# MVPandey/DTS

Measured on AMD Instinct MI355X. Metric: scored_trajectories_per_sec, higher is better.
Workload: dtype bf16

## Files before the change

dts_amd/ops/hip/attention.hip:

```cpp

#include "common.h"
#include "kv_cache.h"
#include <torch/extension.h>
#include <c10/hip/HIPStream.h>
#include <unordered_map>
#include <array>
#include <cstdlib>

using bf16x8 = __attribute__((ext_vector_type(8))) short;
using f32x4 = __attribute__((ext_vector_type(4))) float;
using f32x2 = __attribute__((ext_vector_type(2))) float;
using bf16x2 = __attribute__((ext_vector_type(2))) __bf16;
using u32x2 = __attribute__((ext_vector_type(2))) unsigned int;
using u32x4 = __attribute__((ext_vector_type(4))) unsigned int;


DEV bf16x8 kv_deq8(u32x2 w, float s) {
  union { bf16x2 p[4]; bf16x8 v; } c;
  c.p[0] = __builtin_amdgcn_cvt_scalef32_pk_bf16_fp8(w[0], s, false);
  c.p[1] = __builtin_amdgcn_cvt_scalef32_pk_bf16_fp8(w[0], s, true);
  c.p[2] = __builtin_amdgcn_cvt_scalef32_pk_bf16_fp8(w[1], s, false);
  c.p[3] = __builtin_amdgcn_cvt_scalef32_pk_bf16_fp8(w[1], s, true);
  return c.v;
}


template <int G, int D, typename KV = short>
__global__ void __launch_bounds__(256)
attn_decode_kernel(float* __restrict__ ws_m,
                   float* __restrict__ ws_l,
                   float* __restrict__ ws_o,
                   const short* __restrict__ q,
                   const KV* __restrict__ kcache,
                   const KV* __restrict__ vcache,
                   const int* __restrict__ block_tables,
                   const int* __restrict__ kv_lens,
                   int max_blocks, int Hkv, float scale, long q_tstride,
                   const float* __restrict__ kv_scale) {
  constexpr int BS = 16;
  constexpr int NWAVE = 4;
  constexpr int LPK = 4;
  constexpr int DPL = D / LPK;
  constexpr int DPV = D / WAVE;
  const int seq = blockIdx.x;
  const int kvh = blockIdx.y;
  const int split = blockIdx.z;
  const int S = gridDim.z;
  const int Hq = Hkv * G;
  const int wave = threadIdx.x / WAVE;
  const int lane = threadIdx.x & (WAVE - 1);
  const int kv_len = kv_lens[seq];
  const int n_pages = (kv_len + BS - 1) / BS;
  const int pages_per_split = (n_pages + S - 1) / S;
  const int page_lo = split * pages_per_split;
  const int page_hi = min(n_pages, page_lo + pages_per_split);
  const long ws_base = (((long)seq * Hkv + kvh) * S + split) * G;
  if (page_lo >= page_hi) {
    for (int g = threadIdx.x; g < G; g += blockDim.x) {
      ws_m[ws_base + g] = -1e30f;
      ws_l[ws_base + g] = 0.f;
    }
    return;
  }

  __shared__ float s_scores[NWAVE][G][BS];
  __shared__ float s_m[NWAVE][G], s_l[NWAVE][G];
  __shared__ float s_o[NWAVE][G][D];

  const int c = lane & (LPK - 1);
  const int key_of_lane = lane / LPK;
  int qp_[G][DPL / 2];
#pragma unroll
  for (int g = 0; g < G; ++g) {
    const short* qp = q + (long)seq * q_tstride + (long)(kvh * G + g) * D + c * DPL;
#pragma unroll
    for (int i = 0; i < DPL / 2; ++i) qp_[g][i] = ((const int*)qp)[i];
  }

  float m[G], lsum[G], o[G][DPV];
#pragma unroll
  for (int g = 0; g < G; ++g) {
    m[g] = -1e30f;
    lsum[g] = 0.f;
#pragma unroll
    for (int d = 0; d < DPV; ++d) o[g][d] = 0.f;
  }

  const int* bt = block_tables + (long)seq * max_blocks;

  float sscale = scale;
  if constexpr (sizeof(KV) == 1) {
    if (kv_scale) sscale *= kv_scale[kvh];
  }

  for (int page = page_lo + wave; page < page_hi; page += NWAVE) {
    const long blk = bt[page];
    const KV* kbase =
        kcache + ((blk * Hkv + kvh) * BS) * (long)D;
    const KV* vbase =
        vcache + ((blk * Hkv + kvh) * BS) * (long)D;
    const int valid = min(BS, kv_len - page * BS);

    float partial[G];
#pragma unroll
    for (int g = 0; g < G; ++g) partial[g] = 0.f;
    if constexpr (sizeof(KV) == 1) {
      if (key_of_lane < valid) {
        const KV* kp = kbase + key_of_lane * D + c * DPL;
        unsigned int kw[DPL / 4];
#pragma unroll
        for (int x = 0; x < DPL / 16; ++x) {
          const u32x4 t = ((const u32x4*)kp)[x];
#pragma unroll
          for (int y = 0; y < 4; ++y) kw[4 * x + y] = t[y];
        }
#pragma unroll
        for (int w = 0; w < DPL / 4; ++w) {
          const f32x2 kf[2] = {
              __builtin_amdgcn_cvt_pk_f32_fp8((int)kw[w], false),
              __builtin_amdgcn_cvt_pk_f32_fp8((int)kw[w], true)};
#pragma unroll
          for (int h = 0; h < 2; ++h) {
            const int i = 2 * w + h;
            float k0 = kf[h][0];
            float k1 = kf[h][1];
#pragma unroll
            for (int g = 0; g < G; ++g) {
              float q0 = bf2f((short)(qp_[g][i] & 0xffff));
              float q1 = bf2f((short)((qp_[g][i] >> 16) & 0xffff));
              partial[g] += q0 * k0 + q1 * k1;
            }
          }
        }
      }
    } else if (key_of_lane < valid) {
      const KV* kp = kbase + key_of_lane * D + c * DPL;
#pragma unroll
      for (int i = 0; i < DPL / 2; ++i) {
        int kw = ((const int*)kp)[i];
        float k0 = bf2f((short)(kw & 0xffff));
        float k1 = bf2f((short)((kw >> 16) & 0xffff));
#pragma unroll
        for (int g = 0; g < G; ++g) {
          float q0 = bf2f((short)(qp_[g][i] & 0xffff));
          float q1 = bf2f((short)((qp_[g][i] >> 16) & 0xffff));
          partial[g] += q0 * k0 + q1 * k1;
        }
      }
    }
#pragma unroll
    for (int g = 0; g < G; ++g) {
      partial[g] += __shfl_xor(partial[g], 1, 64);
      partial[g] += __shfl_xor(partial[g], 2, 64);
      if (c == 0)
        s_scores[wave][g][key_of_lane] =
            (key_of_lane < valid) ? partial[g] * sscale : -1e30f;
    }
    asm volatile("s_waitcnt lgkmcnt(0)" ::: "memory");
    __builtin_amdgcn_wave_barrier();

    int vw[BS];
#pragma unroll
    for (int j = 0; j < BS; ++j) {
      if (j < valid) {
        if constexpr (sizeof(KV) == 1) {
          if constexpr (DPV == 2)
            vw[j] = (int)*(const unsigned short*)(vbase + j * D + 2 * lane);
          else
            vw[j] = (int)*(const unsigned char*)(vbase + j * D + lane);
        } else if constexpr (DPV == 2) {
          vw[j] = *(const int*)(vbase + j * D + 2 * lane);
        } else {
          vw[j] = (int)*(const unsigned short*)(vbase + j * D + lane);
        }
      } else {
        vw[j] = 0;
      }
    }

#pragma unroll
    for (int g = 0; g < G; ++g) {
      float tmax = -1e30f;
#pragma unroll
      for (int j = 0; j < BS; ++j) tmax = fmaxf(tmax, s_scores[wave][g][j]);
      float m_new = fmaxf(m[g], tmax);
      if (m_new > -1e30f) {
        float alpha = __expf(m[g] - m_new);
#pragma unroll
        for (int d = 0; d < DPV; ++d) o[g][d] *= alpha;
        lsum[g] *= alpha;
        m[g] = m_new;
        float p[BS];
        float psum = 0.f;
#pragma unroll
        for (int j = 0; j < BS; ++j) {
          p[j] = (j < valid) ? __expf(s_scores[wave][g][j] - m_new) : 0.f;
          psum += p[j];
        }
        lsum[g] += psum;
        if constexpr (sizeof(KV) == 1) {
#pragma unroll
          for (int j = 0; j < BS; ++j) {
            const f32x2 vf = __builtin_amdgcn_cvt_pk_f32_fp8(vw[j], false);
            o[g][0] += p[j] * vf[0];
            if constexpr (DPV == 2) o[g][1] += p[j] * vf[1];
          }
        } else {
#pragma unroll
          for (int j = 0; j < BS; ++j) {
            o[g][0] += p[j] * bf2f((short)(vw[j] & 0xffff));
            if constexpr (DPV == 2)
              o[g][1] += p[j] * bf2f((short)((vw[j] >> 16) & 0xffff));
          }
        }
      }
    }
    __builtin_amdgcn_wave_barrier();
  }

#pragma unroll
  for (int g = 0; g < G; ++g) {
    if (lane == 0) {
      s_m[wave][g] = m[g];
      s_l[wave][g] = lsum[g];
    }
#pragma unroll
    for (int d = 0; d < DPV; ++d) s_o[wave][g][lane * DPV + d] = o[g][d];
  }
  __syncthreads();

  float vscale = 1.f;
  if constexpr (sizeof(KV) == 1) {
    if (kv_scale) vscale = kv_scale[Hkv + kvh];
  }
  const int tid = threadIdx.x;
  for (int gd = tid; gd < G * (D / 2); gd += blockDim.x) {
    const int g = gd / (D / 2);
    const int d0 = (gd % (D / 2)) * 2;
    float m_star = -1e30f;
#pragma unroll
    for (int w = 0; w < NWAVE; ++w) m_star = fmaxf(m_star, s_m[w][g]);
    float l_star = 0.f, acc0 = 0.f, acc1 = 0.f;
#pragma unroll
    for (int w = 0; w < NWAVE; ++w) {
      float f = (s_m[w][g] > -1e30f) ? __expf(s_m[w][g] - m_star) : 0.f;
      l_star += s_l[w][g] * f;
      acc0 += s_o[w][g][d0] * f;
      acc1 += s_o[w][g][d0 + 1] * f;
    }
    if (d0 == 0) {
      ws_m[ws_base + g] = m_star;
      ws_l[ws_base + g] = l_star;
    }
    float* wo = ws_o + (ws_base + g) * D;
    if constexpr (sizeof(KV) == 1) {
      wo[d0] = acc0 * vscale;
      wo[d0 + 1] = acc1 * vscale;
    } else {
      wo[d0] = acc0;
      wo[d0 + 1] = acc1;
    }
  }
}

template <int D>
__global__ void __launch_bounds__(256)
attn_decode_combine(short* __restrict__ out,
                    const float* __restrict__ ws_m,
                    const float* __restrict__ ws_l,
                    const float* __restrict__ ws_o,
                    int S, int G, int Hkv) {
  const int seq = blockIdx.x;
  const int hq = blockIdx.y;
  const int kvh = hq / G;
  const int g = hq % G;
  const int Hq = Hkv * G;
  const long base0 = (((long)seq * Hkv + kvh) * S) * G + g;

  __shared__ float sh_f[64];
  __shared__ float sh_linv[1];
  if (threadIdx.x == 0) {
    float m_star = -1e30f;
    for (int s2 = 0; s2 < S; ++s2)
      m_star = fmaxf(m_star, ws_m[base0 + (long)s2 * G]);
    float l_star = 0.f;
    for (int s2 = 0; s2 < S; ++s2) {
      float mm = ws_m[base0 + (long)s2 * G];
      float f = (mm > -1e30f) ? __expf(mm - m_star) : 0.f;
      sh_f[s2] = f;
      l_star += ws_l[base0 + (long)s2 * G] * f;
    }
    sh_linv[0] = (l_star > 0.f) ? 1.f / l_star : 0.f;
  }
  __syncthreads();
  const float linv = sh_linv[0];
  for (int d = threadIdx.x; d < D; d += blockDim.x) {
    float acc = 0.f;
    for (int s2 = 0; s2 < S; ++s2) {
      float f = sh_f[s2];
      if (f > 0.f) acc += ws_o[(base0 + (long)s2 * G) * D + d] * f;
    }
    out[(((long)seq * Hq) + hq) * D + d] = f2bf(acc * linv);
  }
}


template <int G, int D, int KSTEP>
__global__ void __launch_bounds__(256)
attn_prefill_kernel_v2(short* __restrict__ out,
                       const short* __restrict__ q,
                       const int* __restrict__ cu_q,
                       const long* __restrict__ q_pos,
                       const short* __restrict__ kcache,
                       const short* __restrict__ vcache,
                       const int* __restrict__ block_tables,
                       const int* __restrict__ kv_lens, int max_blocks,
                       int Hkv, float scale, long q_tstride) {
  constexpr int BS = 16;
  constexpr int KCHUNKS = D / 32;
  constexpr int CTILES = D / 16;
  constexpr int LDK = D + 8;
  constexpr int LDV = KSTEP + 4;
  constexpr int ROWS = 64;
  const int POS_PER_WG = ROWS / G;

  const int seq = blockIdx.y;
  const int kvh = blockIdx.z;
  const int Hq = Hkv * G;
  const int q_start = cu_q[seq];
  const int q_len = cu_q[seq + 1] - q_start;
  const int tile = blockIdx.x;
  if (tile * POS_PER_WG >= q_len) return;

  const int wave = threadIdx.x / WAVE;
  const int lane = threadIdx.x & (WAVE - 1);
  const int kv_len = kv_lens[seq];
  const int* bt = block_tables + (long)seq * max_blocks;

  __shared__ short k_lds[KSTEP][LDK];
  __shared__ short v_lds_t[D][LDV];
  __shared__ float s_scores[4][16][KSTEP];
  __shared__ float s_alpha[4][16];
  __shared__ float s_rowl[4][16];
  __shared__ short p_lds[4][16][KSTEP];

  short a_frag[KCHUNKS][8];
  {
    const int r = lane & 15;
    const int row_global = wave * 16 + r;
    const int pos_local = tile * POS_PER_WG + row_global / G;
    const int head = row_global % G;
    const bool valid_row = pos_local < q_len;
    const int tok = q_start + (valid_row ? pos_local : 0);
    const short* qp = q + (long)tok * q_tstride + (long)(kvh * G + head) * D;
#pragma unroll
    for (int kc = 0; kc < KCHUNKS; ++kc) {
      const int kbase = kc * 32 + (lane >> 4) * 8;
      bf16x8 v8 = *(const bf16x8*)(qp + kbase);
#pragma unroll
      for (int i = 0; i < 8; ++i)
        a_frag[kc][i] = valid_row ? v8[i] : (short)0;
    }
  }
  constexpr int SMW = KSTEP / 4;
  const int sm_row = lane / 4;
  const int sm_sub = lane & 3;
  const long sm_pos = tile * POS_PER_WG + (wave * 16 + sm_row) / G;
  const bool sm_valid = sm_pos < q_len;
  const long sm_abs_pos = sm_valid ? q_pos[q_start + sm_pos] : -1;

  f32x4 o_acc[CTILES];
#pragma unroll
  for (int ct = 0; ct < CTILES; ++ct) o_acc[ct] = {0.f, 0.f, 0.f, 0.f};
  float run_m = -1e30f, run_l = 0.f;

  const int last_local_pos = min(q_len, tile * POS_PER_WG + POS_PER_WG) - 1;
  const long last_abs_pos = q_pos[q_start + last_local_pos];
  const int kv_hi = min((long)kv_len, last_abs_pos + 1);

  constexpr int CHUNKS_PT = KSTEP * D / (256 * 8);
  bf16x8 k_stage[CHUNKS_PT], v_stage[CHUNKS_PT];
  int st_key[CHUNKS_PT], st_d0[CHUNKS_PT];

  auto issue_tile = [&](int kv_base) {
#pragma unroll
    for (int c = 0; c < CHUNKS_PT; ++c) {
      const int base = (threadIdx.x + c * 256) * 8;
      const int key = base / D;
      const int d0 = base % D;
      st_key[c] = key;
      st_d0[c] = d0;
      const int kglob = kv_base + key;
      if (kglob < kv_len) {
        const long blk = bt[kglob / BS];
        const long off = ((blk * Hkv + kvh) * BS + kglob % BS) * (long)D + d0;
        k_stage[c] = *(const bf16x8*)(kcache + off);
        v_stage[c] = *(const bf16x8*)(vcache + off);
      } else {
        const bf16x8 z = {0, 0, 0, 0, 0, 0, 0, 0};
        k_stage[c] = z;
        v_stage[c] = z;
      }
    }
  };
  auto write_tile = [&]() {
#pragma unroll
    for (int c = 0; c < CHUNKS_PT; ++c) {
      *(bf16x8*)(&k_lds[st_key[c]][st_d0[c]]) = k_stage[c];
#pragma unroll
      for (int i = 0; i < 8; ++i)
        v_lds_t[st_d0[c] + i][st_key[c]] = v_stage[c][i];
    }
  };

  issue_tile(0);
  write_tile();
  __syncthreads();

  for (int kv_base = 0; kv_base < kv_hi; kv_base += KSTEP) {
    const int kv_next = kv_base + KSTEP;
    if (kv_next < kv_hi) issue_tile(kv_next);

#pragma unroll
    for (int st = 0; st < KSTEP / 16; ++st) {
      f32x4 acc = {0.f, 0.f, 0.f, 0.f};
#pragma unroll
      for (int kc = 0; kc < KCHUNKS; ++kc) {
        const int key = st * 16 + (lane & 15);
        const int d0 = kc * 32 + (lane >> 4) * 8;
        bf16x8 b8 = *(bf16x8*)(&k_lds[key][d0]);
        acc = __builtin_amdgcn_mfma_f32_16x16x32_bf16(
            *(bf16x8*)a_frag[kc], b8, acc, 0, 0, 0);
      }
#pragma unroll
      for (int i = 0; i < 4; ++i) {
        const int row = (lane >> 4) * 4 + i;
        s_scores[wave][row][st * 16 + (lane & 15)] = acc[i] * scale;
      }
    }
    __builtin_amdgcn_s_waitcnt(0);
    __builtin_amdgcn_wave_barrier();

    {
      float tmax = -1e30f;
      float sc[SMW];
#pragma unroll
      for (int jj = 0; jj < SMW; ++jj) {
        const int j = sm_sub * SMW + jj;
        const long key_abs = kv_base + j;
        float s = s_scores[wave][sm_row][j];
        const bool ok =
            sm_valid && key_abs <= sm_abs_pos && key_abs < (long)kv_len;
        sc[jj] = ok ? s : -1e30f;
        tmax = fmaxf(tmax, sc[jj]);
      }
      tmax = fmaxf(tmax, __shfl_xor(tmax, 1, 64));
      tmax = fmaxf(tmax, __shfl_xor(tmax, 2, 64));
      float m_new = fmaxf(run_m, tmax);
      float alpha, rowsum = 0.f;
      if (m_new > -1e30f) {
        alpha = (run_m > -1e30f) ? __expf(run_m - m_new) : 0.f;
#pragma unroll
        for (int jj = 0; jj < SMW; ++jj) {
          float p = (sc[jj] > -1e30f) ? __expf(sc[jj] - m_new) : 0.f;
          p_lds[wave][sm_row][sm_sub * SMW + jj] = f2bf(p);
          rowsum += p;
        }
      } else {
        alpha = 1.f;
#pragma unroll
        for (int jj = 0; jj < SMW; ++jj)
          p_lds[wave][sm_row][sm_sub * SMW + jj] = 0;
      }
      rowsum += __shfl_xor(rowsum, 1, 64);
      rowsum += __shfl_xor(rowsum, 2, 64);
      run_l = run_l * alpha + rowsum;
      run_m = m_new;
      if (sm_sub == 0) {
        s_alpha[wave][sm_row] = alpha;
        s_rowl[wave][sm_row] = run_l;
      }
    }
    __builtin_amdgcn_s_waitcnt(0);
    __builtin_amdgcn_wave_barrier();

    {
      float al[4];
#pragma unroll
      for (int i = 0; i < 4; ++i) al[i] = s_alpha[wave][(lane >> 4) * 4 + i];
      constexpr int HCH = KSTEP / 32;
      bf16x8 pa[HCH];
      {
        const int row = lane & 15;
#pragma unroll
        for (int h = 0; h < HCH; ++h) {
          const int k0 = h * 32 + (lane >> 4) * 8;
#pragma unroll
          for (int i = 0; i < 8; ++i) pa[h][i] = p_lds[wave][row][k0 + i];
        }
      }
#pragma unroll
      for (int ct = 0; ct < CTILES; ++ct) {
#pragma unroll
        for (int i = 0; i < 4; ++i) o_acc[ct][i] *= al[i];
        const int dim = ct * 16 + (lane & 15);
#pragma unroll
        for (int h = 0; h < HCH; ++h) {
          const int kk0 = h * 32 + (lane >> 4) * 8;
          bf16x8 vb;
          ((unsigned long long*)&vb)[0] =
              *(const unsigned long long*)(&v_lds_t[dim][kk0]);
          ((unsigned long long*)&vb)[1] =
              *(const unsigned long long*)(&v_lds_t[dim][kk0 + 4]);
          o_acc[ct] = __builtin_amdgcn_mfma_f32_16x16x32_bf16(
              pa[h], vb, o_acc[ct], 0, 0, 0);
        }
      }
    }
    __syncthreads();
    if (kv_next < kv_hi) {
      write_tile();
      __syncthreads();
    }
  }

  {
    float invl[4];
#pragma unroll
    for (int i = 0; i < 4; ++i) {
      float l = s_rowl[wave][(lane >> 4) * 4 + i];
      invl[i] = (l > 0.f) ? 1.f / l : 0.f;
    }
#pragma unroll
    for (int ct = 0; ct < CTILES; ++ct) {
#pragma unroll
      for (int i = 0; i < 4; ++i) {
        const int row = (lane >> 4) * 4 + i;
        const int row_global = wave * 16 + row;
        const int pos_local = tile * POS_PER_WG + row_global / G;
        if (pos_local >= q_len) continue;
        const int head = row_global % G;
        const int tok = q_start + pos_local;
        const int dim = ct * 16 + (lane & 15);
        out[((long)tok * Hq + kvh * G + head) * D + dim] =
            f2bf(o_acc[ct][i] * invl[i]);
      }
    }
  }
}


template <int G, int D, int KSTEP, typename KV = short>
__global__ void __launch_bounds__(256)
attn_prefill_kernel_v5(short* __restrict__ out,
                       const short* __restrict__ q,
                       const int* __restrict__ cu_q,
                       const long* __restrict__ q_pos,
                       const KV* __restrict__ kcache,
                       const KV* __restrict__ vcache,
                       const int* __restrict__ block_tables,
                       const int* __restrict__ kv_lens, int max_blocks,
                       int Hkv, float scale, long q_tstride,
                       const float* __restrict__ kv_scale) {
  constexpr int BS = 16;
  constexpr int KCHUNKS = D / 32;
  constexpr int CTILES = D / 16;
  constexpr int LDS_PAD = 8;
  constexpr int LDK = D + LDS_PAD;
  constexpr int ROWS = 64;
  const int POS_PER_WG = ROWS / G;

  const int seq = blockIdx.y;
  const int kvh = blockIdx.z;
  const int Hq = Hkv * G;
  const int q_start = cu_q[seq];
  const int q_len = cu_q[seq + 1] - q_start;
  const int tile = blockIdx.x;
  if (tile * POS_PER_WG >= q_len) return;

  const int wave = threadIdx.x / WAVE;
  const int lane = threadIdx.x & (WAVE - 1);
  const int kv_len = kv_lens[seq];
  const int* bt = block_tables + (long)seq * max_blocks;

  __shared__ short k_lds[KSTEP][LDK];
  __shared__ short v_lds[KSTEP][LDK];

  float k_scale = 1.f, v_scale = 1.f;
  if constexpr (sizeof(KV) == 1) {
    if (kv_scale) {
      k_scale = kv_scale[kvh];
      v_scale = kv_scale[Hkv + kvh];
    }
  }

  short q_frag[KCHUNKS][8];
  {
    const int r = lane & 15;
    const int row_global = wave * 16 + r;
    const int pos_local = tile * POS_PER_WG + row_global / G;
    const int head = row_global % G;
    const bool valid_row = pos_local < q_len;
    const int tok = q_start + (valid_row ? pos_local : 0);
    const short* qp = q + (long)tok * q_tstride + (long)(kvh * G + head) * D;
#pragma unroll
    for (int kc = 0; kc < KCHUNKS; ++kc) {
      const int kbase = kc * 32 + (lane >> 4) * 8;
      bf16x8 v8 = *(const bf16x8*)(qp + kbase);
#pragma unroll
      for (int i = 0; i < 8; ++i)
        q_frag[kc][i] = valid_row ? v8[i] : (short)0;
    }
  }
  const int my_q = lane & 15;
  const int my_row_global = wave * 16 + my_q;
  const long my_pos_local = tile * POS_PER_WG + my_row_global / G;
  const bool my_valid = my_pos_local < q_len;
  const long my_abs_pos = my_valid ? q_pos[q_start + my_pos_local] : -1;

  f32x4 o_acc[CTILES];
#pragma unroll
  for (int ct = 0; ct < CTILES; ++ct) o_acc[ct] = {0.f, 0.f, 0.f, 0.f};
  float run_m = -1e30f, run_l = 0.f;

  const int last_local_pos = min(q_len, tile * POS_PER_WG + POS_PER_WG) - 1;
  const long last_abs_pos = q_pos[q_start + last_local_pos];
  const int kv_hi = min((long)kv_len, last_abs_pos + 1);

  for (int kv_base = 0; kv_base < kv_hi; kv_base += KSTEP) {
    {
      const int elems = KSTEP * D;
      for (int base = threadIdx.x * 8; base < elems; base += 256 * 8) {
        const int key = base / D;
        const int d0 = base % D;
        const int kglob = kv_base + key;
        if (kglob < kv_len) {
          const long blk = bt[kglob / BS];
          const long off =
              ((blk * Hkv + kvh) * BS + kglob % BS) * (long)D + d0;
          if constexpr (sizeof(KV) == 1) {
            *(bf16x8*)(&k_lds[key][d0]) =
                kv_deq8(*(const u32x2*)(kcache + off), k_scale);
            *(bf16x8*)(&v_lds[key][d0]) =
                kv_deq8(*(const u32x2*)(vcache + off), v_scale);
          } else {
            *(bf16x8*)(&k_lds[key][d0]) = *(const bf16x8*)(kcache + off);
            *(bf16x8*)(&v_lds[key][d0]) = *(const bf16x8*)(vcache + off);
          }
        } else {
          const bf16x8 z = {0, 0, 0, 0, 0, 0, 0, 0};
          *(bf16x8*)(&k_lds[key][d0]) = z;
          *(bf16x8*)(&v_lds[key][d0]) = z;
        }
      }
    }
    __syncthreads();

    constexpr int STILES = KSTEP / 16;
    f32x4 sc[STILES];
#pragma unroll
    for (int st = 0; st < STILES; ++st) {
      f32x4 acc = {0.f, 0.f, 0.f, 0.f};
#pragma unroll
      for (int kc = 0; kc < KCHUNKS; ++kc) {
        const int key = st * 16 + (lane & 15);
        const int d0 = kc * 32 + (lane >> 4) * 8;
        bf16x8 k8 = *(bf16x8*)(&k_lds[key][d0]);
        acc = __builtin_amdgcn_mfma_f32_16x16x32_bf16(
            k8, *(bf16x8*)q_frag[kc], acc, 0, 0, 0);
      }
      sc[st] = acc;
    }

    float p[STILES][4];
    float tmax = -1e30f;
#pragma unroll
    for (int st = 0; st < STILES; ++st)
#pragma unroll
      for (int i = 0; i < 4; ++i) {
        const long key_abs = kv_base + st * 16 + (lane >> 4) * 4 + i;
        const bool ok =
            my_valid && key_abs <= my_abs_pos && key_abs < (long)kv_len;
        p[st][i] = ok ? sc[st][i] * scale : -1e30f;
        tmax = fmaxf(tmax, p[st][i]);
      }
    tmax = fmaxf(tmax, __shfl_xor(tmax, 16, 64));
    tmax = fmaxf(tmax, __shfl_xor(tmax, 32, 64));
    const float m_new = fmaxf(run_m, tmax);
    float alpha;
    float rowsum = 0.f;
    if (m_new > -1e30f) {
      alpha = (run_m > -1e30f) ? __expf(run_m - m_new) : 0.f;
#pragma unroll
      for (int st = 0; st < STILES; ++st)
#pragma unroll
        for (int i = 0; i < 4; ++i) {
          p[st][i] = (p[st][i] > -1e30f) ? __expf(p[st][i] - m_new) : 0.f;
          rowsum += p[st][i];
        }
    } else {
      alpha = 1.f;
#pragma unroll
      for (int st = 0; st < STILES; ++st)
#pragma unroll
        for (int i = 0; i < 4; ++i) p[st][i] = 0.f;
    }
    rowsum += __shfl_xor(rowsum, 16, 64);
    rowsum += __shfl_xor(rowsum, 32, 64);
    run_l = run_l * alpha + rowsum;
    run_m = m_new;

    unsigned int ppack[STILES][2];
#pragma unroll
    for (int st = 0; st < STILES; ++st) {
#pragma unroll
      for (int hpair = 0; hpair < 2; ++hpair) {
        const unsigned int lo =
            (unsigned short)f2bf(p[st][hpair * 2]);
        const unsigned int hi =
            (unsigned short)f2bf(p[st][hpair * 2 + 1]);
        ppack[st][hpair] = lo | (hi << 16);
      }
    }
    constexpr int HCH = KSTEP / 32;
    bf16x8 pa[HCH];
#pragma unroll
    for (int h = 0; h < HCH; ++h) {
      const int kb = 8 * (lane >> 4);
      const int st_a = h * 2 + kb / 16;
      const int ga = (kb % 16) / 4;
      const int st_b = h * 2 + (kb + 4) / 16;
      const int gb = ((kb + 4) % 16) / 4;
      unsigned int paw[4];
#pragma unroll
      for (int pr = 0; pr < 2; ++pr) {
        unsigned int va = 0, vb2 = 0;
#pragma unroll
        for (int st = 0; st < STILES; ++st) {
          const unsigned int ta =
              (unsigned int)__shfl((int)ppack[st][pr], (ga << 4) | my_q, 64);
          const unsigned int tb =
              (unsigned int)__shfl((int)ppack[st][pr], (gb << 4) | my_q, 64);
          if (st == st_a) va = ta;
          if (st == st_b) vb2 = tb;
        }
        paw[pr] = va;
        paw[2 + pr] = vb2;
      }
#pragma unroll
      for (int j = 0; j < 4; ++j) {
        pa[h][2 * j] = (short)(paw[j] & 0xffff);
        pa[h][2 * j + 1] = (short)(paw[j] >> 16);
      }
    }
#pragma unroll
    for (int ct = 0; ct < CTILES; ++ct) {
#pragma unroll
      for (int i = 0; i < 4; ++i) {
        const float al = __shfl(alpha, (lane >> 4) * 4 + i, 64);
        o_acc[ct][i] *= al;
      }
    }
#pragma unroll
    for (int ct = 0; ct < CTILES; ++ct) {
      const int dim = ct * 16 + (lane & 15);
#pragma unroll
      for (int h = 0; h < HCH; ++h) {
        bf16x8 vb;
        const int kk0 = h * 32 + (lane >> 4) * 8;
#pragma unroll
        for (int i = 0; i < 8; ++i) vb[i] = v_lds[kk0 + i][dim];
        o_acc[ct] = __builtin_amdgcn_mfma_f32_16x16x32_bf16(
            pa[h], vb, o_acc[ct], 0, 0, 0);
      }
    }
    __syncthreads();
  }

  {
#pragma unroll
    for (int ct = 0; ct < CTILES; ++ct) {
#pragma unroll
      for (int i = 0; i < 4; ++i) {
        const int row = (lane >> 4) * 4 + i;
        const float l = __shfl(run_l, row, 64);
        const float invl = (l > 0.f) ? 1.f / l : 0.f;
        const int row_global = wave * 16 + row;
        const int pos_local = tile * POS_PER_WG + row_global / G;
        if (pos_local >= q_len) continue;
        const int head = row_global % G;
        const int tok = q_start + pos_local;
        const int dim = ct * 16 + (lane & 15);
        out[((long)tok * Hq + kvh * G + head) * D + dim] =
            f2bf(o_acc[ct][i] * invl);
      }
    }
  }
}


template <int G, int D, bool SWZ, typename KV = short>
__global__ void __launch_bounds__(256)
attn_prefill_kernel(short* __restrict__ out,
                    const short* __restrict__ q,
                    const int* __restrict__ cu_q,
                    const long* __restrict__ q_pos,
                    const KV* __restrict__ kcache,
                    const KV* __restrict__ vcache,
                    const int* __restrict__ block_tables,
                    const int* __restrict__ kv_lens, int max_blocks, int Hkv,
                    float scale, long q_tstride,
                    const float* __restrict__ kv_scale) {
  constexpr int BS = 16;
  constexpr int KSTEP = 32;
  constexpr int KCHUNKS = D / 32;
  constexpr int CTILES = D / 16;
  constexpr int LDS_PAD = 8;
  constexpr int LDK = D + LDS_PAD;
  constexpr int ROWS = 64;
  const int POS_PER_WG = ROWS / G;

  const int seq = blockIdx.y;
  const int kvh = blockIdx.z;
  const int Hq = Hkv * G;
  const int q_start = cu_q[seq];
  const int q_len = cu_q[seq + 1] - q_start;
  const int tile = blockIdx.x;
  if (tile * POS_PER_WG >= q_len) return;

  const int wave = threadIdx.x / WAVE;
  const int lane = threadIdx.x & (WAVE - 1);
  const int kv_len = kv_lens[seq];
  const int* bt = block_tables + (long)seq * max_blocks;

  __shared__ short k_lds[KSTEP][LDK];
  __shared__ short v_lds[KSTEP][LDK];
  float k_scale = 1.f, v_scale = 1.f;
  if constexpr (sizeof(KV) == 1) {
    if (kv_scale) {
      k_scale = kv_scale[kvh];
      v_scale = kv_scale[Hkv + kvh];
    }
  }
  auto swz_col = [](int key, int col) -> int {
    if constexpr (SWZ) return ((col & ~7) ^ ((key & 7) << 3)) | (col & 7);
    else return col;
  };
  __shared__ float s_scores[4][16][KSTEP];
  __shared__ float s_alpha[4][16];
  __shared__ float s_rowl[4][16];
  __shared__ short p_lds[4][16][KSTEP];

  long my_pos[4];
  short a_frag[KCHUNKS][8];
  {
    const int r = lane & 15;
    const int row_global = wave * 16 + r;
    const int pos_local = tile * POS_PER_WG + row_global / G;
    const int head = row_global % G;
    const bool valid_row = pos_local < q_len;
    const int tok = q_start + (valid_row ? pos_local : 0);
    const short* qp = q + (long)tok * q_tstride + (long)(kvh * G + head) * D;
#pragma unroll
    for (int kc = 0; kc < KCHUNKS; ++kc) {
      const int kbase = kc * 32 + (lane >> 4) * 8;
      bf16x8 v8 = *(const bf16x8*)(qp + kbase);
#pragma unroll
      for (int i = 0; i < 8; ++i)
        a_frag[kc][i] = valid_row ? v8[i] : (short)0;
    }
  }
  const int sm_row = lane / 4;
  const int sm_sub = lane & 3;
  const long sm_pos =
      tile * POS_PER_WG + (wave * 16 + sm_row) / G;
  const bool sm_valid = sm_pos < q_len;
  const long sm_abs_pos = sm_valid ? q_pos[q_start + sm_pos] : -1;

  f32x4 o_acc[CTILES];
#pragma unroll
  for (int ct = 0; ct < CTILES; ++ct) o_acc[ct] = {0.f, 0.f, 0.f, 0.f};
  float run_m = -1e30f, run_l = 0.f;

  const int last_local_pos = min(q_len, tile * POS_PER_WG + POS_PER_WG) - 1;
  const long last_abs_pos = q_pos[q_start + last_local_pos];
  const int kv_hi = min((long)kv_len, last_abs_pos + 1);

  for (int kv_base = 0; kv_base < kv_hi; kv_base += KSTEP) {
    {
      const int elems = KSTEP * D;
      for (int base = threadIdx.x * 8; base < elems; base += 256 * 8) {
        const int key = base / D;
        const int d0 = base % D;
        const int page = kv_base / BS + key / BS;
        const int koff = key % BS;
        const int kglob = kv_base + key;
        const int dst = swz_col(key, d0);
        if (kglob < kv_len) {
          const long blk = bt[page];
          const KV* kp =
              kcache + ((blk * Hkv + kvh) * BS + koff) * (long)D + d0;
          const KV* vp =
              vcache + ((blk * Hkv + kvh) * BS + koff) * (long)D + d0;
          if constexpr (sizeof(KV) == 1) {
            *(bf16x8*)(&k_lds[key][dst]) = kv_deq8(*(const u32x2*)kp, k_scale);
            *(bf16x8*)(&v_lds[key][dst]) = kv_deq8(*(const u32x2*)vp, v_scale);
          } else {
            *(bf16x8*)(&k_lds[key][dst]) = *(const bf16x8*)kp;
            *(bf16x8*)(&v_lds[key][dst]) = *(const bf16x8*)vp;
          }
        } else {
          bf16x8 z = {0, 0, 0, 0, 0, 0, 0, 0};
          *(bf16x8*)(&k_lds[key][dst]) = z;
          *(bf16x8*)(&v_lds[key][dst]) = z;
        }
      }
    }
    __syncthreads();

#pragma unroll
    for (int st = 0; st < 2; ++st) {
      f32x4 acc = {0.f, 0.f, 0.f, 0.f};
#pragma unroll
      for (int kc = 0; kc < KCHUNKS; ++kc) {
        const int key = st * 16 + (lane & 15);
        const int d0 = kc * 32 + (lane >> 4) * 8;
        bf16x8 b8 = *(const bf16x8*)(&k_lds[key][swz_col(key, d0)]);
        acc = __builtin_amdgcn_mfma_f32_16x16x32_bf16(
            *(bf16x8*)a_frag[kc], b8, acc, 0, 0, 0);
      }
#pragma unroll
      for (int i = 0; i < 4; ++i) {
        const int row = (lane >> 4) * 4 + i;
        s_scores[wave][row][st * 16 + (lane & 15)] = acc[i] * scale;
      }
    }
    __builtin_amdgcn_s_waitcnt(0);
    __builtin_amdgcn_wave_barrier();

    {
      float tmax = -1e30f;
      float sc[8];
#pragma unroll
      for (int jj = 0; jj < 8; ++jj) {
        const int j = sm_sub * 8 + jj;
        const long key_abs = kv_base + j;
        float s = s_scores[wave][sm_row][j];
        const bool ok = sm_valid && key_abs <= sm_abs_pos &&
                        key_abs < (long)kv_len;
        sc[jj] = ok ? s : -1e30f;
        tmax = fmaxf(tmax, sc[jj]);
      }
      tmax = fmaxf(tmax, __shfl_xor(tmax, 1, 64));
      tmax = fmaxf(tmax, __shfl_xor(tmax, 2, 64));
      float m_new = fmaxf(run_m, tmax);
      float alpha, rowsum = 0.f;
      if (m_new > -1e30f) {
        alpha = (run_m > -1e30f) ? __expf(run_m - m_new) : 0.f;
#pragma unroll
        for (int jj = 0; jj < 8; ++jj) {
          float p = (sc[jj] > -1e30f) ? __expf(sc[jj] - m_new) : 0.f;
          p_lds[wave][sm_row][sm_sub * 8 + jj] = f2bf(p);
          rowsum += p;
        }
      } else {
        alpha = 1.f;
#pragma unroll
        for (int jj = 0; jj < 8; ++jj)
          p_lds[wave][sm_row][sm_sub * 8 + jj] = 0;
      }
      rowsum += __shfl_xor(rowsum, 1, 64);
      rowsum += __shfl_xor(rowsum, 2, 64);
      run_l = run_l * alpha + rowsum;
      run_m = m_new;
      if (sm_sub == 0) {
        s_alpha[wave][sm_row] = alpha;
        s_rowl[wave][sm_row] = run_l;
      }
    }
    __builtin_amdgcn_s_waitcnt(0);
    __builtin_amdgcn_wave_barrier();

    {
      float al[4];
#pragma unroll
      for (int i = 0; i < 4; ++i) al[i] = s_alpha[wave][(lane >> 4) * 4 + i];
      bf16x8 pa0, pa1;
      {
        const int row = lane & 15;
        const int k0 = (lane >> 4) * 8;
#pragma unroll
        for (int i = 0; i < 8; ++i) pa0[i] = p_lds[wave][row][k0 + i];
        pa1 = pa0;
      }
#pragma unroll
      for (int ct = 0; ct < CTILES; ++ct) {
#pragma unroll
        for (int i = 0; i < 4; ++i) o_acc[ct][i] *= al[i];
        bf16x8 vb;
        const int dim = ct * 16 + (lane & 15);
        const int kk0 = (lane >> 4) * 8;
#pragma unroll
        for (int i = 0; i < 8; ++i)
          vb[i] = v_lds[kk0 + i][swz_col(kk0 + i, dim)];
        o_acc[ct] = __builtin_amdgcn_mfma_f32_16x16x32_bf16(pa0, vb,
                                                            o_acc[ct], 0, 0, 0);
      }
    }
    __syncthreads();
  }

  {
    float invl[4];
#pragma unroll
    for (int i = 0; i < 4; ++i) {
      float l = s_rowl[wave][(lane >> 4) * 4 + i];
      invl[i] = (l > 0.f) ? 1.f / l : 0.f;
    }
#pragma unroll
    for (int ct = 0; ct < CTILES; ++ct) {
#pragma unroll
      for (int i = 0; i < 4; ++i) {
        const int row = (lane >> 4) * 4 + i;
        const int row_global = wave * 16 + row;
        const int pos_local = tile * POS_PER_WG + row_global / G;
        if (pos_local >= q_len) continue;
        const int head = row_global % G;
        const int tok = q_start + pos_local;
        const int dim = ct * 16 + (lane & 15);
        out[((long)tok * Hq + kvh * G + head) * D + dim] =
            f2bf(o_acc[ct][i] * invl[i]);
      }
    }
  }
}


void attn_decode_paged(torch::Tensor out, torch::Tensor q,
                       torch::Tensor kcache, torch::Tensor vcache,
                       torch::Tensor block_tables, torch::Tensor kv_lens,
                       double scale, c10::optional<torch::Tensor> kv_scale) {
  const int B = q.size(0), Hq = q.size(1), D = q.size(2);
  const int Hkv = kcache.size(1);
  const int G = Hq / Hkv;
  const int max_blocks = block_tables.size(1);
  TORCH_CHECK(kcache.size(2) == 16, "block_size must be 16");
  const bool fp8 = kv_cache_is_fp8(kcache, vcache);
  const float* kv_scale_p = kv_scale_ptr(kv_scale, kcache, fp8);
  TORCH_CHECK(block_tables.scalar_type() == torch::kInt32);
  TORCH_CHECK(q.stride(2) == 1 && q.stride(1) == D, "q heads must be dense");
  TORCH_CHECK(out.is_contiguous(), "out must be contiguous");
  const long q_tstride = q.stride(0);
  static const int S = [] {
    const char* e = getenv("DTS_DECODE_SPLITS");
    int v = e ? atoi(e) : 8;
    return (v >= 1 && v <= 64) ? v : 8;
  }();
  static std::unordered_map<std::string, std::array<torch::Tensor, 3>> ws_cache;
  const std::string key = std::to_string(q.get_device()) + ":" +
                          std::to_string(B) + ":" + std::to_string(Hkv) + ":" +
                          std::to_string(G) + ":" + std::to_string(D);
  auto it = ws_cache.find(key);
  if (it == ws_cache.end()) {
    auto f32 =
        torch::TensorOptions().dtype(torch::kFloat32).device(q.device());
    it = ws_cache
             .emplace(key,
                      std::array<torch::Tensor, 3>{
                          torch::empty({B, Hkv, S, G}, f32),
                          torch::empty({B, Hkv, S, G}, f32),
                          torch::empty({(long)B, Hkv, S, G, D}, f32)})
             .first;
  }
  torch::Tensor ws_m = it->second[0];
  torch::Tensor ws_l = it->second[1];
  torch::Tensor ws_o = it->second[2];
  dim3 grid(B, Hkv, S);
  dim3 block(256);
  auto stream = c10::hip::getCurrentHIPStream();
#define DECODE_LAUNCH(g, d, kv)                                              \
  hipLaunchKernelGGL((attn_decode_kernel<g, d, kv>), grid, block, 0, stream, \
                     (float*)ws_m.data_ptr(), (float*)ws_l.data_ptr(),       \
                     (float*)ws_o.data_ptr(), (const short*)q.data_ptr(),    \
                     (const kv*)kcache.data_ptr(),                           \
                     (const kv*)vcache.data_ptr(),                           \
                     (const int*)block_tables.data_ptr(),                    \
                     (const int*)kv_lens.data_ptr(), max_blocks, Hkv,        \
                     (float)scale, q_tstride, kv_scale_p)
#define DECODE_CASE(g, d)                                                    \
  do {                                                                       \
    if (fp8) DECODE_LAUNCH(g, d, unsigned char);                             \
    else DECODE_LAUNCH(g, d, short);                                         \
    hipLaunchKernelGGL((attn_decode_combine<d>), dim3(B, Hq), dim3(256), 0,  \
                       stream, (short*)out.data_ptr(),                       \
                       (const float*)ws_m.data_ptr(),                        \
                       (const float*)ws_l.data_ptr(),                        \
                       (const float*)ws_o.data_ptr(), S, G, Hkv);            \
  } while (0)
  if (D == 128 && G == 4) DECODE_CASE(4, 128);
  else if (D == 128 && G == 8) DECODE_CASE(8, 128);
  else if (D == 128 && G == 1) DECODE_CASE(1, 128);
  else if (D == 64 && G == 1) DECODE_CASE(1, 64);
  else TORCH_CHECK(false, "unsupported decode attn shape D=", D, " G=", G);
#undef DECODE_CASE
#undef DECODE_LAUNCH
  HIP_CHECK_LAST();
}

void attn_prefill_paged(torch::Tensor out, torch::Tensor q, torch::Tensor cu_q,
                        torch::Tensor q_pos, torch::Tensor kcache,
                        torch::Tensor vcache, torch::Tensor block_tables,
                        torch::Tensor kv_lens, double scale, int64_t swz,
                        c10::optional<torch::Tensor> kv_scale) {
  if (swz < 0) {
    static int env_v = [] {
      const char* e = getenv("DTS_PREFILL_V");
      return e ? atoi(e) : -1;
    }();
    swz = (env_v >= 0) ? env_v : 5;
  }
  const bool fp8 = kv_cache_is_fp8(kcache, vcache);
  TORCH_CHECK(!fp8 || swz == 0 || swz == 4 || swz == 5,
              "prefill variant ", swz, " (DTS_PREFILL_V) does not support an "
              "FP8 KV cache; use 0, 4 or 5");
  const float* kv_scale_p = kv_scale_ptr(kv_scale, kcache, fp8);
  const int Hq = q.size(1), D = q.size(2);
  const int Hkv = kcache.size(1);
  const int G = Hq / Hkv;
  const int P = cu_q.size(0) - 1;
  const int max_blocks = block_tables.size(1);
  TORCH_CHECK(q.stride(2) == 1 && q.stride(1) == D, "q heads must be dense");
  TORCH_CHECK(out.is_contiguous(), "out must be contiguous");
  const long q_tstride = q.stride(0);
  TORCH_CHECK(D == 128 || D == 64, "prefill kernel supports head_dim 64/128");
  TORCH_CHECK(kcache.size(2) == 16, "block_size must be 16");
  TORCH_CHECK(cu_q.scalar_type() == torch::kInt32);
  const long Tq = q.size(0);
  const int pos_per_wg = 64 / G;
  const int max_tiles = (int)((Tq + pos_per_wg - 1) / pos_per_wg);
  dim3 grid(max_tiles, P, Hkv);
  dim3 block(256);
  auto stream = c10::hip::getCurrentHIPStream();
#define PREFILL_CASE(g, d)                                                    \
  do {                                                                        \
    if (swz == 2)                                                             \
      hipLaunchKernelGGL((attn_prefill_kernel_v2<g, d, 64>), grid, block, 0,  \
                         stream, (short*)out.data_ptr(),                      \
                         (const short*)q.data_ptr(),                          \
                         (const int*)cu_q.data_ptr(),                         \
                         (const long*)q_pos.data_ptr(),                       \
                         (const short*)kcache.data_ptr(),                     \
                         (const short*)vcache.data_ptr(),                     \
                         (const int*)block_tables.data_ptr(),                 \
                         (const int*)kv_lens.data_ptr(), max_blocks, Hkv,     \
                         (float)scale, q_tstride);                            \
    else if (swz == 3)                                                        \
      hipLaunchKernelGGL((attn_prefill_kernel_v2<g, d, 32>), grid, block, 0,  \
                         stream, (short*)out.data_ptr(),                      \
                         (const short*)q.data_ptr(),                          \
                         (const int*)cu_q.data_ptr(),                         \
                         (const long*)q_pos.data_ptr(),                       \
                         (const short*)kcache.data_ptr(),                     \
                         (const short*)vcache.data_ptr(),                     \
                         (const int*)block_tables.data_ptr(),                 \
                         (const int*)kv_lens.data_ptr(), max_blocks, Hkv,     \
                         (float)scale, q_tstride);                            \
    else if (swz == 4)                                                        \
      hipLaunchKernelGGL((attn_prefill_kernel_v5<g, d, 32>), grid, block, 0,  \
                         stream, (short*)out.data_ptr(),                      \
                         (const short*)q.data_ptr(),                         \
                         (const int*)cu_q.data_ptr(),                         \
                         (const long*)q_pos.data_ptr(),                       \
                         (const short*)kcache.data_ptr(),                     \
                         (const short*)vcache.data_ptr(),                     \
                         (const int*)block_tables.data_ptr(),                 \
                         (const int*)kv_lens.data_ptr(), max_blocks, Hkv,     \
                         (float)scale, q_tstride, nullptr);                   \
    else if (swz == 5)                                                        \
      hipLaunchKernelGGL((attn_prefill_kernel_v5<g, d, 64>), grid, block, 0,  \
                         stream, (short*)out.data_ptr(),                      \
                         (const short*)q.data_ptr(),                         \
                         (const int*)cu_q.data_ptr(),                         \
                         (const long*)q_pos.data_ptr(),                       \
                         (const short*)kcache.data_ptr(),                     \
                         (const short*)vcache.data_ptr(),                     \
                         (const int*)block_tables.data_ptr(),                 \
                         (const int*)kv_lens.data_ptr(), max_blocks, Hkv,     \
                         (float)scale, q_tstride, nullptr);                   \
    else if (swz == 1)                                                        \
      hipLaunchKernelGGL((attn_prefill_kernel<g, d, true>), grid, block, 0,   \
                         stream, (short*)out.data_ptr(),                      \
                         (const short*)q.data_ptr(),                          \
                         (const int*)cu_q.data_ptr(),                         \
                         (const long*)q_pos.data_ptr(),                       \
                         (const short*)kcache.data_ptr(),                     \
                         (const short*)vcache.data_ptr(),                     \
                         (const int*)block_tables.data_ptr(),                 \
                         (const int*)kv_lens.data_ptr(), max_blocks, Hkv,     \
                         (float)scale, q_tstride, nullptr);                   \
    else                                                                      \
      hipLaunchKernelGGL((attn_prefill_kernel<g, d, false>), grid, block, 0,  \
                         stream, (short*)out.data_ptr(),                      \
                         (const short*)q.data_ptr(),                          \
                         (const int*)cu_q.data_ptr(),                         \
                         (const long*)q_pos.data_ptr(),                       \
                         (const short*)kcache.data_ptr(),                     \
                         (const short*)vcache.data_ptr(),                     \
                         (const int*)block_tables.data_ptr(),                 \
                         (const int*)kv_lens.data_ptr(), max_blocks, Hkv,     \
                         (float)scale, q_tstride, nullptr);                   \
  } while (0)
#define PREFILL_LAUNCH_FP8(kern)                                              \
  hipLaunchKernelGGL(kern, grid, block, 0, stream, (short*)out.data_ptr(),    \
                     (const short*)q.data_ptr(), (const int*)cu_q.data_ptr(), \
                     (const long*)q_pos.data_ptr(),                           \
                     (const unsigned char*)kcache.data_ptr(),                 \
                     (const unsigned char*)vcache.data_ptr(),                 \
                     (const int*)block_tables.data_ptr(),                     \
                     (const int*)kv_lens.data_ptr(), max_blocks, Hkv,         \
                     (float)scale, q_tstride, kv_scale_p)
#define PREFILL_CASE_FP8(g, d)                                                \
  do {                                                                        \
    if (swz == 4)                                                             \
      PREFILL_LAUNCH_FP8((attn_prefill_kernel_v5<g, d, 32, unsigned char>));  \
    else if (swz == 5)                                                        \
      PREFILL_LAUNCH_FP8((attn_prefill_kernel_v5<g, d, 64, unsigned char>));  \
    else                                                                      \
      PREFILL_LAUNCH_FP8((attn_prefill_kernel<g, d, false, unsigned char>));  \
  } while (0)
  if (fp8) {
    if (D == 128 && G == 4) PREFILL_CASE_FP8(4, 128);
    else if (D == 128 && G == 8) PREFILL_CASE_FP8(8, 128);
    else if (D == 128 && G == 1) PREFILL_CASE_FP8(1, 128);
    else if (D == 128 && G == 2) PREFILL_CASE_FP8(2, 128);
    else if (D == 64 && G == 1) PREFILL_CASE_FP8(1, 64);
    else TORCH_CHECK(false, "unsupported prefill shape G=", G, " D=", D);
  } else if (D == 128 && G == 4) PREFILL_CASE(4, 128);
  else if (D == 128 && G == 8) PREFILL_CASE(8, 128);
  else if (D == 128 && G == 1) PREFILL_CASE(1, 128);
  else if (D == 128 && G == 2) PREFILL_CASE(2, 128);
  else if (D == 64 && G == 1) PREFILL_CASE(1, 64);
  else TORCH_CHECK(false, "unsupported prefill shape G=", G, " D=", D);
#undef PREFILL_CASE
#undef PREFILL_CASE_FP8
#undef PREFILL_LAUNCH_FP8
  HIP_CHECK_LAST();
}
```

Baseline: 0.3868.

## Add v6 prefill attention kernel with register prefetch and transposed LDS V reads

Adds a new paged prefill attention kernel, v6, and makes it the default variant. It double-buffers KV tile loads through registers: the next tile's global loads and block-table lookups are issued before the current tile's compute, and the data is committed to LDS afterward. V is stored in grouped LDS rows and read with ds_read_tr16_b64 transpose loads instead of element-wise gathers. This hides global memory latency and cuts LDS read instructions, at the cost of more registers per thread and a second sync per iteration.

```diff
diff --git a/dts_amd/ops/hip/attention.hip b/dts_amd/ops/hip/attention.hip
--- a/dts_amd/ops/hip/attention.hip
+++ b/dts_amd/ops/hip/attention.hip
@@ -775,6 +775,334 @@
       }
     }
     __syncthreads();
+  }
+
+  {
+#pragma unroll
+    for (int ct = 0; ct < CTILES; ++ct) {
+#pragma unroll
+      for (int i = 0; i < 4; ++i) {
+        const int row = (lane >> 4) * 4 + i;
+        const float l = __shfl(run_l, row, 64);
+        const float invl = (l > 0.f) ? 1.f / l : 0.f;
+        const int row_global = wave * 16 + row;
+        const int pos_local = tile * POS_PER_WG + row_global / G;
+        if (pos_local >= q_len) continue;
+        const int head = row_global % G;
+        const int tok = q_start + pos_local;
+        const int dim = ct * 16 + (lane & 15);
+        out[((long)tok * Hq + kvh * G + head) * D + dim] =
+            f2bf(o_acc[ct][i] * invl);
+      }
+    }
+  }
+}
+
+
+typedef short i16x4 __attribute__((ext_vector_type(4)));
+typedef __attribute__((address_space(3))) i16x4 lds_i16x4;
+
+template <int G, int D, int KSTEP, typename KV = short, bool PF = false>
+__global__ void __launch_bounds__(256)
+attn_prefill_kernel_v6(short* __restrict__ out,
+                       const short* __restrict__ q,
+                       const int* __restrict__ cu_q,
+                       const long* __restrict__ q_pos,
+                       const KV* __restrict__ kcache,
+                       const KV* __restrict__ vcache,
+                       const int* __restrict__ block_tables,
+                       const int* __restrict__ kv_lens, int max_blocks,
+                       int Hkv, float scale, long q_tstride,
+                       const float* __restrict__ kv_scale) {
+  static_assert(KSTEP == 64, "v6 is built for 64-key tiles");
+  constexpr int BS = 16;
+  constexpr int KCHUNKS = D / 32;
+  constexpr int CTILES = D / 16;
+  constexpr int LDS_PAD = 8;
+  constexpr int LDK = D + LDS_PAD;
+  constexpr int LDV = D + 16;
+  constexpr int VGRP = 8 * LDV + 64;
+  constexpr int ROWS = 64;
+  constexpr int NIT = KSTEP * D / (256 * 8);
+  constexpr int KEYS_PER_IT = 256 * 8 / D;
+  constexpr bool FP8 = sizeof(KV) == 1;
+  const int POS_PER_WG = ROWS / G;
+
+  const int seq = blockIdx.y;
+  const int kvh = blockIdx.z;
+  const int Hq = Hkv * G;
+  const int q_start = cu_q[seq];
+  const int q_len = cu_q[seq + 1] - q_start;
+  const int tile = blockIdx.x;
+  if (tile * POS_PER_WG >= q_len) return;
+
+  const int wave = threadIdx.x / WAVE;
+  const int lane = threadIdx.x & (WAVE - 1);
+  const int kv_len = kv_lens[seq];
+  const int* bt = block_tables + (long)seq * max_blocks;
+
+  __shared__ __attribute__((aligned(16))) short k_lds[KSTEP][LDK];
+  __shared__ __attribute__((aligned(16))) short v_lds[(KSTEP / 8) * VGRP];
+  auto v_off = [](int key, int col) -> int {
+    return (key >> 3) * VGRP + (key & 7) * LDV + col;
+  };
+
+  float k_scale = 1.f, v_scale = 1.f;
+  if constexpr (FP8) {
+    if (kv_scale) {
+      k_scale = kv_scale[kvh];
+      v_scale = kv_scale[Hkv + kvh];
+    }
+  }
+
+  short q_frag[KCHUNKS][8];
+  {
+    const int r = lane & 15;
+    const int row_global = wave * 16 + r;
+    const int pos_local = tile * POS_PER_WG + row_global / G;
+    const int head = row_global % G;
+    const bool valid_row = pos_local < q_len;
+    const int tok = q_start + (valid_row ? pos_local : 0);
+    const short* qp = q + (long)tok * q_tstride + (long)(kvh * G + head) * D;
+#pragma unroll
+    for (int kc = 0; kc < KCHUNKS; ++kc) {
+      const int kbase = kc * 32 + (lane >> 4) * 8;
+      bf16x8 v8 = *(const bf16x8*)(qp + kbase);
+#pragma unroll
+      for (int i = 0; i < 8; ++i)
+        q_frag[kc][i] = valid_row ? v8[i] : (short)0;
+    }
+  }
+  const int my_q = lane & 15;
+  const int my_row_global = wave * 16 + my_q;
+  const long my_pos_local = tile * POS_PER_WG + my_row_global / G;
+  const bool my_valid = my_pos_local < q_len;
+  const long my_abs_pos = my_valid ? q_pos[q_start + my_pos_local] : -1;
+
+  f32x4 o_acc[CTILES];
+#pragma unroll
+  for (int ct = 0; ct < CTILES; ++ct) o_acc[ct] = {0.f, 0.f, 0.f, 0.f};
+  float run_m = -1e30f, run_l = 0.f;
+
+  const int last_local_pos = min(q_len, tile * POS_PER_WG + POS_PER_WG) - 1;
+  const long last_abs_pos = q_pos[q_start + last_local_pos];
+  const int kv_hi = min((long)kv_len, last_abs_pos + 1);
+
+  const int ld_key = threadIdx.x * 8 / D;
+  const int ld_d0 = threadIdx.x * 8 % D;
+  const short* v_rd =
+      &v_lds[v_off(8 * (lane >> 4) + ((lane >> 2) & 3), 4 * (lane & 3))];
+
+  using stage_t = typename std::conditional<FP8, u32x2, bf16x8>::type;
+  stage_t kreg[NIT], vreg[NIT];
+  int blk_next[NIT];
+  auto fetch_bt = [&](int base) {
+#pragma unroll
+    for (int it = 0; it < NIT; ++it) {
+      const int kg = min(base + ld_key + it * KEYS_PER_IT, kv_len - 1);
+      blk_next[it] = bt[kg / BS];
+    }
+  };
+  auto issue_tile = [&](int base) {
+#pragma unroll
+    for (int it = 0; it < NIT; ++it) {
+      const int kg = min(base + ld_key + it * KEYS_PER_IT, kv_len - 1);
+      const long off =
+          (((long)blk_next[it] * Hkv + kvh) * BS + kg % BS) * (long)D + ld_d0;
+      kreg[it] = *(const stage_t*)(kcache + off);
+      vreg[it] = *(const stage_t*)(vcache + off);
+    }
+  };
+  auto commit_tile = [&](int base) {
+#pragma unroll
+    for (int it = 0; it < NIT; ++it) {
+      const int key = ld_key + it * KEYS_PER_IT;
+      const bool live = base + key < kv_len;
+      bf16x8 k8, v8;
+      if constexpr (FP8) {
+        k8 = kv_deq8(kreg[it], k_scale);
+        v8 = kv_deq8(vreg[it], v_scale);
+      } else {
+        k8 = kreg[it];
+        v8 = vreg[it];
+      }
+      const bf16x8 z = {0, 0, 0, 0, 0, 0, 0, 0};
+      *(bf16x8*)(&k_lds[key][ld_d0]) = live ? k8 : z;
+      *(bf16x8*)(&v_lds[v_off(key, ld_d0)]) = live ? v8 : z;
+    }
+  };
+
+  if constexpr (PF) {
+    if (kv_hi > 0) {
+      fetch_bt(0);
+      issue_tile(0);
+      if (KSTEP < kv_hi) fetch_bt(KSTEP);
+      commit_tile(0);
+      __syncthreads();
+    }
+  }
+
+  for (int kv_base = 0; kv_base < kv_hi; kv_base += KSTEP) {
+    if constexpr (PF) {
+      if (kv_base + KSTEP < kv_hi) {
+        issue_tile(kv_base + KSTEP);
+        if (kv_base + 2 * KSTEP < kv_hi) fetch_bt(kv_base + 2 * KSTEP);
+      }
+    } else {
+      const int elems = KSTEP * D;
+      for (int base = threadIdx.x * 8; base < elems; base += 256 * 8) {
+        const int key = base / D;
+        const int d0 = base % D;
+        const int kglob = kv_base + key;
+        if (kglob < kv_len) {
+          const long blk = bt[kglob / BS];
+          const long off =
+              ((blk * Hkv + kvh) * BS + kglob % BS) * (long)D + d0;
+          if constexpr (sizeof(KV) == 1) {
+            *(bf16x8*)(&k_lds[key][d0]) =
+                kv_deq8(*(const u32x2*)(kcache + off), k_scale);
+            *(bf16x8*)(&v_lds[v_off(key, d0)]) =
+                kv_deq8(*(const u32x2*)(vcache + off), v_scale);
+          } else {
+            *(bf16x8*)(&k_lds[key][d0]) = *(const bf16x8*)(kcache + off);
+            *(bf16x8*)(&v_lds[v_off(key, d0)]) =
+                *(const bf16x8*)(vcache + off);
+          }
+        } else {
+          const bf16x8 z = {0, 0, 0, 0, 0, 0, 0, 0};
+          *(bf16x8*)(&k_lds[key][d0]) = z;
+          *(bf16x8*)(&v_lds[v_off(key, d0)]) = z;
+        }
+      }
+      __syncthreads();
+    }
+
+    constexpr int STILES = KSTEP / 16;
+    f32x4 sc[STILES];
+#pragma unroll
+    for (int st = 0; st < STILES; ++st) {
+      f32x4 acc = {0.f, 0.f, 0.f, 0.f};
+#pragma unroll
+      for (int kc = 0; kc < KCHUNKS; ++kc) {
+        const int key = st * 16 + (lane & 15);
+        const int d0 = kc * 32 + (lane >> 4) * 8;
+        bf16x8 k8 = *(bf16x8*)(&k_lds[key][d0]);
+        acc = __builtin_amdgcn_mfma_f32_16x16x32_bf16(
+            k8, *(bf16x8*)q_frag[kc], acc, 0, 0, 0);
+      }
+      sc[st] = acc;
+    }
+
+    float p[STILES][4];
+    float tmax = -1e30f;
+#pragma unroll
+    for (int st = 0; st < STILES; ++st)
+#pragma unroll
+      for (int i = 0; i < 4; ++i) {
+        const long key_abs = kv_base + st * 16 + (lane >> 4) * 4 + i;
+        const bool ok =
+            my_valid && key_abs <= my_abs_pos && key_abs < (long)kv_len;
+        p[st][i] = ok ? sc[st][i] * scale : -1e30f;
+        tmax = fmaxf(tmax, p[st][i]);
+      }
+    tmax = fmaxf(tmax, __shfl_xor(tmax, 16, 64));
+    tmax = fmaxf(tmax, __shfl_xor(tmax, 32, 64));
+    const float m_new = fmaxf(run_m, tmax);
+    float alpha;
+    float rowsum = 0.f;
+    if (m_new > -1e30f) {
+      alpha = (run_m > -1e30f) ? __expf(run_m - m_new) : 0.f;
+#pragma unroll
+      for (int st = 0; st < STILES; ++st)
+#pragma unroll
+        for (int i = 0; i < 4; ++i) {
+          p[st][i] = (p[st][i] > -1e30f) ? __expf(p[st][i] - m_new) : 0.f;
+          rowsum += p[st][i];
+        }
+    } else {
+      alpha = 1.f;
+#pragma unroll
+      for (int st = 0; st < STILES; ++st)
+#pragma unroll
+        for (int i = 0; i < 4; ++i) p[st][i] = 0.f;
+    }
+    rowsum += __shfl_xor(rowsum, 16, 64);
+    rowsum += __shfl_xor(rowsum, 32, 64);
+    run_l = run_l * alpha + rowsum;
+    run_m = m_new;
+
+    unsigned int ppack[STILES][2];
+#pragma unroll
+    for (int st = 0; st < STILES; ++st) {
+#pragma unroll
+      for (int hpair = 0; hpair < 2; ++hpair) {
+        const unsigned int lo =
+            (unsigned short)f2bf(p[st][hpair * 2]);
+        const unsigned int hi =
+            (unsigned short)f2bf(p[st][hpair * 2 + 1]);
+        ppack[st][hpair] = lo | (hi << 16);
+      }
+    }
+    constexpr int HCH = KSTEP / 32;
+    bf16x8 pa[HCH];
+#pragma unroll
+    for (int h = 0; h < HCH; ++h) {
+      const int kb = 8 * (lane >> 4);
+      const int st_a = h * 2 + kb / 16;
+      const int ga = (kb % 16) / 4;
+      const int st_b = h * 2 + (kb + 4) / 16;
+      const int gb = ((kb + 4) % 16) / 4;
+      unsigned int paw[4];
+#pragma unroll
+      for (int pr = 0; pr < 2; ++pr) {
+        unsigned int va = 0, vb2 = 0;
+#pragma unroll
+        for (int st = 0; st < STILES; ++st) {
+          const unsigned int ta =
+              (unsigned int)__shfl((int)ppack[st][pr], (ga << 4) | my_q, 64);
+          const unsigned int tb =
+              (unsigned int)__shfl((int)ppack[st][pr], (gb << 4) | my_q, 64);
+          if (st == st_a) va = ta;
+          if (st == st_b) vb2 = tb;
+        }
+        paw[pr] = va;
+        paw[2 + pr] = vb2;
+      }
+#pragma unroll
+      for (int j = 0; j < 4; ++j) {
+        pa[h][2 * j] = (short)(paw[j] & 0xffff);
+        pa[h][2 * j + 1] = (short)(paw[j] >> 16);
+      }
+    }
+#pragma unroll
+    for (int ct = 0; ct < CTILES; ++ct) {
+#pragma unroll
+      for (int i = 0; i < 4; ++i) {
+        const float al = __shfl(alpha, (lane >> 4) * 4 + i, 64);
+        o_acc[ct][i] *= al;
+      }
+    }
+#pragma unroll
+    for (int ct = 0; ct < CTILES; ++ct) {
+#pragma unroll
+      for (int h = 0; h < HCH; ++h) {
+        const short* vp = v_rd + h * 4 * VGRP + ct * 16;
+        const i16x4 lo =
+            __builtin_amdgcn_ds_read_tr16_b64_v4i16((lds_i16x4*)vp);
+        const i16x4 hi = __builtin_amdgcn_ds_read_tr16_b64_v4i16(
+            (lds_i16x4*)(vp + 4 * LDV));
+        const bf16x8 vb = __builtin_shufflevector(lo, hi, 0, 1, 2, 3, 4, 5, 6, 7);
+        o_acc[ct] = __builtin_amdgcn_mfma_f32_16x16x32_bf16(
+            pa[h], vb, o_acc[ct], 0, 0, 0);
+      }
+    }
+    __syncthreads();
+    if constexpr (PF) {
+      if (kv_base + KSTEP < kv_hi) {
+        commit_tile(kv_base + KSTEP);
+        __syncthreads();
+      }
+    }
   }
 
   {
@@ -1117,12 +1445,13 @@
       const char* e = getenv("DTS_PREFILL_V");
       return e ? atoi(e) : -1;
     }();
-    swz = (env_v >= 0) ? env_v : 5;
+    swz = (env_v >= 0) ? env_v : 6;
   }
   const bool fp8 = kv_cache_is_fp8(kcache, vcache);
-  TORCH_CHECK(!fp8 || swz == 0 || swz == 4 || swz == 5,
+  const bool v6 = swz == 6 || swz == 7;
+  TORCH_CHECK(!fp8 || swz == 0 || swz == 4 || swz == 5 || v6,
               "prefill variant ", swz, " (DTS_PREFILL_V) does not support an "
-              "FP8 KV cache; use 0, 4 or 5");
+              "FP8 KV cache; use 0, 4, 5, 6 or 7");
   const float* kv_scale_p = kv_scale_ptr(kv_scale, kcache, fp8);
   const int Hq = q.size(1), D = q.size(2);
   const int Hkv = kcache.size(1);
@@ -1141,9 +1470,23 @@
   dim3 grid(max_tiles, P, Hkv);
   dim3 block(256);
   auto stream = c10::hip::getCurrentHIPStream();
+  const bool v6_pf = swz == 6;
+#define PREFILL_LAUNCH_BF16(kern)                                             \
+  hipLaunchKernelGGL(kern, grid, block, 0, stream, (short*)out.data_ptr(),    \
+                     (const short*)q.data_ptr(), (const int*)cu_q.data_ptr(), \
+                     (const long*)q_pos.data_ptr(),                           \
+                     (const short*)kcache.data_ptr(),                         \
+                     (const short*)vcache.data_ptr(),                         \
+                     (const int*)block_tables.data_ptr(),                     \
+                     (const int*)kv_lens.data_ptr(), max_blocks, Hkv,         \
+                     (float)scale, q_tstride, nullptr)
 #define PREFILL_CASE(g, d)                                                    \
   do {                                                                        \
-    if (swz == 2)                                                             \
+    if (v6 && v6_pf)                                                          \
+      PREFILL_LAUNCH_BF16((attn_prefill_kernel_v6<g, d, 64, short, true>));   \
+    else if (v6)                                                              \
+      PREFILL_LAUNCH_BF16((attn_prefill_kernel_v6<g, d, 64, short, false>));  \
+    else if (swz == 2)                                                        \
       hipLaunchKernelGGL((attn_prefill_kernel_v2<g, d, 64>), grid, block, 0,  \
                          stream, (short*)out.data_ptr(),                      \
                          (const short*)q.data_ptr(),                          \
@@ -1221,7 +1564,13 @@
                      (float)scale, q_tstride, kv_scale_p)
 #define PREFILL_CASE_FP8(g, d)                                                \
   do {                                                                        \
-    if (swz == 4)                                                             \
+    if (v6 && v6_pf)                                                          \
+      PREFILL_LAUNCH_FP8(                                                     \
+          (attn_prefill_kernel_v6<g, d, 64, unsigned char, true>));           \
+    else if (v6)                                                              \
+      PREFILL_LAUNCH_FP8(                                                     \
+          (attn_prefill_kernel_v6<g, d, 64, unsigned char, false>));          \
+    else if (swz == 4)                                                        \
       PREFILL_LAUNCH_FP8((attn_prefill_kernel_v5<g, d, 32, unsigned char>));  \
     else if (swz == 5)                                                        \
       PREFILL_LAUNCH_FP8((attn_prefill_kernel_v5<g, d, 64, unsigned char>));  \
@@ -1244,5 +1593,6 @@
 #undef PREFILL_CASE
 #undef PREFILL_CASE_FP8
 #undef PREFILL_LAUNCH_FP8
+#undef PREFILL_LAUNCH_BF16
   HIP_CHECK_LAST();
 }
```

After: 0.4274, median of 6. 1.11x the previous value.
